# TinyMPC/TinyMPC

Hardware: AMD Instinct MI355X
Metric: QP solves/sec (+ ADMM iters/sec), 64k-batch quadrotor hover (higher is better)
Workload: dtype f64; 1 GPU; quadrotor_hovering (nx=12, nu=4, N=10), 65536 identical instances per GPU, closed-loop MPC steps from a cold start (BASELINE configs[1]); batch_per_gpu=65536, total_batch=65536, parallelism=batch-sharded x1, mpc_steps_per_launch=8, stats_exchange=none (one rank), launcher=plain process

## Files before the change

tinympc_amd/csrc/admm_kernel.hip.h:

```cpp
#pragma once
#include <hip/hip_runtime.h>
#include <stdint.h>

namespace tinympc_amd {

enum : int {
    TAB_MB = 0,
    TAB_MF1 = 256,
    TAB_MF2 = 512,
    TAB_PT = 768,
    TAB_VEC = 1024,
    TAB_BOUNDS = 1024 + 16 * 16,
};
enum : int {
    VEC_CB = 0,
    VEC_CF = 1,
    VEC_QR = 2,
    VEC_SMASK = 3,
    VEC_NIM = 4,
    VEC_SOCFLAG = 5,
    VEC_CONE_BASE = 6,
    VEC_CONE_MU = 7,
    VEC_LINFLAG = 9,
    VEC_TLINFLAG = 10,
// ... 133 lines not shown
        ring1<0, NA>(a0, srcA, mA);
        ring1<NA, NB>(a0, srcB, mB);
        return a0;
    } else {
        double a0 = init, a1 = 0.0;
        ring<MODE, 0, NA>(a0, a1, srcA, mA);
        ring<MODE, NA, NB>(a0, a1, srcB, mB);
        return a0 + a1;
    }
}
template <int MODE, int COL0, int NCOL>
__device__ __forceinline__ double ring_sum(double init, double src, const double* m) {
    if constexpr (MODE == 2) {
        double a0 = init;
        ring1<COL0, NCOL>(a0, src, m);
        return a0;
    } else {
        double a0 = init, a1 = 0.0;
        ring<MODE, COL0, NCOL>(a0, a1, src, m);
        return a0 + a1;
    }
}
template <int MODE, int COL0, int NCOL>
__device__ __forceinline__ double ring_short(double init, double src, const double* m) {
    if constexpr (MODE == 1) return ring_sum<1, COL0, NCOL>(init, src, m);
    else { double a0 = init; ring1<COL0, NCOL>(a0, src, m); return a0; }
}


#define RINGH_LO(k, p) DPP_FMA("a0", "src", "m" #k, "%[c0]+" #k, "0x3")
#define RINGH_HI(k, p) DPP_FMA("a0", "src", "m" #k, "8+%[c0]+" #k, "0xc")
#define RINGH_CASE(K)                                                                                                                    \
    if constexpr (NCOL == K)                                                                                                             \
        asm("s_nop 1\n\t" DPP_REP(K, RINGH_LO) "s_nop 0\n\t" DPP_REP(K, RINGH_HI) : [a0] "+&v"(a0) : [src] "v"(src), [c0] "i"(COL0) DPP_REP(K, DPP_ROW_M));
template <int COL0, int NCOL>
__device__ __forceinline__ void ring1_half(double& a0, double src, const double* m) {
    static_assert(NCOL >= 1 && COL0 + NCOL <= 8, "one half row");
    RINGH_CASE(1) RINGH_CASE(2) RINGH_CASE(3) RINGH_CASE(4) RINGH_CASE(5) RINGH_CASE(6) RINGH_CASE(7) RINGH_CASE(8)
}


#if defined(TINYMPC_FUSED_NX) && defined(TINYMPC_FUSED_NU)
#define TINYMPC_FUSED 1
constexpr bool fused_shape(int na, int nb) { return na == TINYMPC_FUSED_NX && nb == TINYMPC_FUSED_NU; }
#define FUSED_ROW_OPERANDS [c0] "i"(TINYMPC_FUSED_NX) DPP_REP(TINYMPC_FUSED_NX, DPP_ROW_A) DPP_REP(TINYMPC_FUSED_NU, DPP_ROW_B)
#else
constexpr bool fused_shape(int, int) { return false; }
#endif
#define BWD_COL_A(k, p) DPP_FMA("acc", "sa", "a" #k, #k, "0xf")
#define BWD_COL_B(k, p) DPP_FMA("acc", "sb", "b" #k, "%[c0]+" #k, "0xf")
#define FWD_COL_A(k, p) DPP_FMA("t", "xi", "a" #k, #k, "0xf")
#define FWD_COL_B(k, p) DPP_FMA("xn", "t", "b" #k, "%[c0]+" #k, "0xf")
#define FWD_COL_B_INPLACE(k, p) DPP_FMA("t", "t", "b" #k, "%[c0]+" #k, "%[bm]")
template <int NA, int NB>
__device__ __forceinline__ void fused_backward_step(double& qlo, double& acc, double vn, double g, double qx, double rho, double smask, double cb,
                                                    double sa, double sb, const double* ma, const double* mb_) {
#ifdef TINYMPC_FUSED
    if constexpr (fused_shape(NA, NB)) {
        double tmp;
        asm("v_add_f64 %[tmp], %[vn], -%[g]\n\t"
            "v_fma_f64 %[qlo], -%[rho], %[tmp], %[qx]\n\t"
            "v_fma_f64 %[acc], %[qlo], %[smask], %[cb]\n\t"
            DPP_REP(TINYMPC_FUSED_NX, BWD_COL_A) DPP_REP(TINYMPC_FUSED_NU, BWD_COL_B)
            : [qlo] "=&v"(qlo), [acc] "=&v"(acc), [tmp] "=&v"(tmp)
            : [vn] "v"(vn), [g] "v"(g), [qx] "v"(qx), [rho] "v"(rho), [smask] "v"(smask), [cb] "v"(cb), [sa] "v"(sa), [sb] "v"(sb), FUSED_ROW_OPERANDS);
    }
#endif
}
template <int NA, int NB>
__device__ __forceinline__ void fused_backward_step_soc(double& qlo, double& acc, double vn, double g, double qx, double w, double rho,
                                                        double smask, double cb, double sa, double sb, const double* ma, const double* mb_) {
#ifdef TINYMPC_FUSED
    if constexpr (fused_shape(NA, NB)) {
        double tmp;
        asm("v_add_f64 %[tmp], %[vn], -%[g]\n\t"
            "v_fma_f64 %[qlo], -%[rho], %[tmp], %[qx]\n\t"
            "v_fma_f64 %[qlo], -%[rho], %[w], %[qlo]\n\t"
            "v_fma_f64 %[acc], %[qlo], %[smask], %[cb]\n\t"
            DPP_REP(TINYMPC_FUSED_NX, BWD_COL_A) DPP_REP(TINYMPC_FUSED_NU, BWD_COL_B)
            : [qlo] "=&v"(qlo), [acc] "=&v"(acc), [tmp] "=&v"(tmp)
            : [vn] "v"(vn), [g] "v"(g), [qx] "v"(qx), [rho] "v"(rho), [smask] "v"(smask), [cb] "v"(cb), [sa] "v"(sa), [sb] "v"(sb),
              [w] "v"(w), FUSED_ROW_OPERANDS);
    }
#endif
}
template <int NA, int NB, bool INPLACE = false>
__device__ __forceinline__ void fused_forward_step(double& tt, double& vn, double& t, double& xn, double xi, double g, double lo, double hi,
                                                   const double* ma, const double* mb_) {
#ifdef TINYMPC_FUSED
    if constexpr (fused_shape(NA, NB) && !(INPLACE && TINYMPC_FUSED_NX % 4 == 0)) {
        double vm;
        asm("v_add_f64 %[tt], %[xi], %[g]\n\t"
            "v_max_f64 %[vm], %[lo], %[tt]\n\t"
            DPP_REP(TINYMPC_FUSED_NX, FWD_COL_A)
            "v_min_f64 %[vn], %[hi], %[vm]\n\t"
            "v_mov_b64 %[xn], %[t]\n\t"
            DPP_REP(TINYMPC_FUSED_NU, FWD_COL_B)
            : [tt] "=&v"(tt), [vm] "=&v"(vm), [vn] "=&v"(vn), [xn] "=&v"(xn), [t] "+&v"(t)
            : [xi] "v"(xi), [g] "v"(g), [lo] "v"(lo), [hi] "v"(hi), FUSED_ROW_OPERANDS);
    }
    if constexpr (fused_shape(NA, NB) && INPLACE && TINYMPC_FUSED_NX % 4 == 0) {
        asm("v_add_f64 %[tt], %[xi], %[g]\n\t"
            DPP_REP(TINYMPC_FUSED_NX, FWD_COL_A)
            "v_max_f64 %[vn], %[lo], %[tt]\n\t"
            "v_min_f64 %[vn], %[hi], %[vn]\n\t"
            DPP_REP(TINYMPC_FUSED_NU, FWD_COL_B_INPLACE)
            : [tt] "=&v"(tt), [vn] "=&v"(vn), [t] "+&v"(t)
            : [xi] "v"(xi), [g] "v"(g), [lo] "v"(lo), [hi] "v"(hi), [bm] "i"((1 << (TINYMPC_FUSED_NX / 4)) - 1), FUSED_ROW_OPERANDS);
        xn = t;
    }
#endif
}
#if defined(TINYMPC_FUSED) && TINYMPC_FUSED_NX + TINYMPC_FUSED_NU <= 8
#define TINYMPC_FUSED_HALF 1
#endif
#define HBWD_COL_A_LO(k, p) DPP_FMA("acc", "sa", "a" #k, #k, "0x3")
#define HBWD_COL_A_HI(k, p) DPP_FMA("acc", "sa", "a" #k, "8+" #k, "0xc")
#define HBWD_COL_B_LO(k, p) DPP_FMA("acc", "sb", "b" #k, "%[c0]+" #k, "0x3")
// ... 5 lines not shown
template <int NA, int NB>
__device__ __forceinline__ void fused_backward_step_half(double& qlo, double& acc, double& dnp, double& tmpn, double tmp, double vnn, double gn, double qx,
                                                         double rho, double smask, double cb, double nim, double cf, double sa, double sb,
                                                         const double* ma, const double* mb_) {
#ifdef TINYMPC_FUSED_HALF
    if constexpr (fused_shape(NA, NB)) {
        asm("v_fma_f64 %[qlo], -%[rho], %[tmp], %[qx]\n\t"
            "v_fma_f64 %[acc], %[qlo], %[smask], %[cb]\n\t"
            "v_fma_f64 %[dnp], %[sa], %[nim], %[cf]\n\t"
            DPP_REP(TINYMPC_FUSED_NX, HBWD_COL_A_LO) DPP_REP(TINYMPC_FUSED_NU, HBWD_COL_B_LO)
            "v_add_f64 %[tmpn], %[vnn], -%[gn]\n\t"
            DPP_REP(TINYMPC_FUSED_NX, HBWD_COL_A_HI) DPP_REP(TINYMPC_FUSED_NU, HBWD_COL_B_HI)
            : [qlo] "=&v"(qlo), [acc] "=&v"(acc), [dnp] "=&v"(dnp), [tmpn] "=&v"(tmpn)
            : [tmp] "v"(tmp), [vnn] "v"(vnn), [gn] "v"(gn), [qx] "v"(qx), [rho] "v"(rho), [smask] "v"(smask), [cb] "v"(cb),
              [nim] "v"(nim), [cf] "v"(cf), [sa] "v"(sa), [sb] "v"(sb), FUSED_ROW_OPERANDS);
    }
#endif
}
template <int NA, int NB>
__device__ __forceinline__ void fused_forward_step_half(double& tt, double& vn, double& t, double& xn, double& gnew, double xi, double g,
                                                        double lo, double hi, const double* ma, const double* mb_) {
#ifdef TINYMPC_FUSED_HALF
    if constexpr (fused_shape(NA, NB)) {
        double vm;
        asm("v_add_f64 %[tt], %[xi], %[g]\n\t"
            "v_max_f64 %[vm], %[lo], %[tt]\n\t"
            DPP_REP(TINYMPC_FUSED_NX, HFWD_COL_A_LO)
            "v_min_f64 %[vn], %[hi], %[vm]\n\t"
            DPP_REP(TINYMPC_FUSED_NX, HFWD_COL_A_HI)
            "v_mov_b64 %[xn], %[t]\n\t"
            "v_add_f64 %[gnew], %[tt], -%[vn]\n\t"
            DPP_REP(TINYMPC_FUSED_NU, HFWD_COL_B_LO)
            "s_nop 0\n\t"
            DPP_REP(TINYMPC_FUSED_NU, HFWD_COL_B_HI)
            : [tt] "=&v"(tt), [vm] "=&v"(vm), [vn] "=&v"(vn), [xn] "=&v"(xn), [t] "+&v"(t), [gnew] "=&v"(gnew)
            : [xi] "v"(xi), [g] "v"(g), [lo] "v"(lo), [hi] "v"(hi), FUSED_ROW_OPERANDS);
    }
#endif
}

__device__ __forceinline__ double vmax64(double a, double b) {
    double r;
    asm("v_max_f64 %0, %1, %2" : "=v"(r) : "v"(a), "v"(b));
    return r;
}
__device__ __forceinline__ double vmin64(double a, double b) {
    double r;
    asm("v_min_f64 %0, %1, %2" : "=v"(r) : "v"(a), "v"(b));
    return r;
}
__device__ __forceinline__ double pinned_sub64(double a, double b) {
    double r = a - b;
    asm volatile("" : "+v"(r));
    return r;
}
__device__ __forceinline__ double vclamp64(double lo, double hi, double t) {
    double r;
    asm("v_max_f64 %0, %1, %2\n\tv_min_f64 %0, %3, %0" : "=&v"(r) : "v"(lo), "v"(t), "v"(hi));
    return r;
}

__device__ __forceinline__ double vmax_abs64(double a, double b) {
    double r;
    asm("v_max_f64 %0, %1, |%2|" : "=v"(r) : "v"(a), "v"(b));
    return r;
}
template <bool OPAQUE>
__device__ __forceinline__ double resid_max(double a, double b) {
    if constexpr (OPAQUE) return vmax_abs64(a, b);
    else return fmax(a, fabs(b));
}

#ifndef TINYMPC_PRIM_STORE
#define TINYMPC_PRIM_STORE 1
#endif
#ifndef TINYMPC_REF_LOAD
#define TINYMPC_REF_LOAD 1
#endif
#ifndef TINYMPC_FULL_LINE_STORES
#define TINYMPC_FULL_LINE_STORES 2
#endif
__device__ __forceinline__ double load_ref(const double* p) {
#if TINYMPC_REF_LOAD == 1
    return __builtin_nontemporal_load(p);
#else
    return *p;
#endif
}
__device__ __forceinline__ void store_primal(double* p, double v) {
#if TINYMPC_PRIM_STORE == 1
    __builtin_nontemporal_store(v, p);
#elif TINYMPC_PRIM_STORE == 2
    asm volatile("global_store_dwordx2 %0, %1, off sc1" : : "v"(p), "v"(v) : "memory");
#elif TINYMPC_PRIM_STORE == 3
    asm volatile("global_store_dwordx2 %0, %1, off sc0 sc1" : : "v"(p), "v"(v) : "memory");
#elif TINYMPC_PRIM_STORE == 4
    asm volatile("global_store_dwordx2 %0, %1, off sc0 sc1 nt" : : "v"(p), "v"(v) : "memory");
#else
    *p = v;
#endif
}

__device__ __forceinline__ double grp_max16(double v) {
#pragma unroll
    for (int off = 8; off >= 1; off >>= 1) v = fmax(v, __shfl_xor(v, off, 16));
    return v;
// ... 169 lines not shown
        socmask = P.tab[TAB_VEC + VEC_SOCFLAG * 16 + j];
        soc_lane = socmask != 0.0;
        cone_base = (int)P.tab[TAB_VEC + VEC_CONE_BASE * 16 + j];
        cone_c = (cone_base >= 0) ? (j - cone_base) : 0;
        proj_lane = soc_lane && cone_base >= 0;
    }
    constexpr int SOC_PASSES = SOC ? (soc_item_passes(NX, NU, N) > 0 ? soc_item_passes(NX, NU, N) : 1) : 1;
    int item_at[SOC_PASSES];
    float item_mu[SOC_PASSES], item_rmu[SOC_PASSES];
    bool mu_pow2 = true;
    int soc_passes = 0;
    if constexpr (SOC) {
        if (lane < 3) {
            sC[4 * N * SLOT_D + lane] = lane == 2 ? 1.0 : 0.0;
            sC[4 * N * SLOT_D + PL_GC + lane] = 0.0;
            sC[4 * N * SLOT_D + PL_VC + lane] = lane == 2 ? 1.0 : 0.0;
        }
        const unsigned heads = (unsigned)(__builtin_amdgcn_ballot_w64(proj_lane && cone_c == 0) & 0xFFFFull);
#pragma unroll
        for (int p = 0; p < SOC_PASSES; ++p) {
            int t = p * 16 + j;
            item_at[p] = 4 * N * SLOT_D; item_mu[p] = 1.0f;
            if (heads && p * 16 < soc_items_of(heads, NX, N)) soc_passes = p + 1;
            for (unsigned m = heads; m; m &= m - 1) {
                const int hb = __builtin_ctz(m);
                const int cnt = hb < NX ? N : N - 1;
                if (t >= 0 && t < cnt) {
                    item_at[p] = (grp * N + t + (hb < NX ? 0 : 1)) * SLOT_D + hb;
                    item_mu[p] = (float)P.tab[TAB_VEC + VEC_CONE_MU * 16 + hb];
                    t = -1;
                } else if (t >= 0) t -= cnt;
            }
            item_rmu[p] = 1.0f / item_mu[p];
            const unsigned mb_ = __float_as_uint(item_mu[p]);
            const bool p2 = (mb_ & 0x807FFFFFu) == 0u && (mb_ >> 23) >= 127u - 60u && (mb_ >> 23) <= 127u + 60u;
            if (__builtin_amdgcn_ballot_w64(!p2) != 0ull) mu_pow2 = false;
        }
    }
    bool lin_lane = false, tlin_lane = false;
    if constexpr (LS) lin_lane = P.tab[TAB_VEC + VEC_LINFLAG * 16 + j] != 0.0;
    if constexpr (LT) tlin_lane = P.tab[TAB_VEC + VEC_TLINFLAG * 16 + j] != 0.0;
    constexpr bool LPL = solve_kernel_lin_planes(NX, NU, N, SOC, LIN, KMAX, UB);
    constexpr bool LSP = LS && LPL, LTP = LT && LPL, LSR = LS && !LPL, LTR = LT && !LPL;
    constexpr int CSL = LPL ? ((NZ + 1) | 1) : 1;
    __shared__ double sLV[LSP ? 4 * N * CSL : 1], sLG[LSP ? 4 * N * CSL : 1];
    __shared__ double sTV[LTP ? 4 * N * CSL : 1], sTG[LTP ? 4 * N * CSL : 1];
    double ones[(LSR || LTR) ? 16 : 1];
#pragma unroll
    for (int k = 0; k < ((LSR || LTR) ? 16 : 1); ++k) ones[k] = 1.0;
    bool lin_x_on = false, lin_u_on = false, tlin_x_on = false, tlin_u_on = false;
    if constexpr (LS) { lin_x_on = P.tab[TAB_VEC + VEC_LINFLAG * 16] != 0.0; lin_u_on = P.tab[TAB_VEC + VEC_LINFLAG * 16 + NX] != 0.0; }
    if constexpr (LT) { tlin_x_on = P.tab[TAB_VEC + VEC_TLINFLAG * 16] != 0.0; tlin_u_on = P.tab[TAB_VEC + VEC_TLINFLAG * 16 + NX] != 0.0; }
    double rho = P.rho;
    __builtin_amdgcn_fence(__ATOMIC_RELEASE, "wavefront");
    __builtin_amdgcn_wave_barrier();

    const double lo_u = P.tab[TAB_BOUNDS + (N > 1 ? 16 : 0) + j], hi_u = P.tab[TAB_BOUNDS + N * 16 + (N > 1 ? 16 : 0) + j];
    const double lo_u0 = P.tab[TAB_BOUNDS + j], hi_u0 = P.tab[TAB_BOUNDS + N * 16 + j];
    const int ninst = PF ? P.batch : (P.index ? *P.count : (P.perm ? P.perm_count : P.batch));
    const int ntiles = (ninst + IPW - 1) / IPW;
    const bool resumed = !PF && P.index != nullptr;
    const bool has_traj = !PF && P.traj != nullptr;
    extern __shared__ __attribute__((aligned(16))) double sPF[];
    typedef const __attribute__((address_space(1))) void* pf_gptr;
    typedef __attribute__((address_space(3))) void* pf_lptr;
    constexpr int PF_S0 = 128, PF_S1 = PF_S0 + PF_ARR, PF_S2 = PF_S1 + PF_ARR, PF_S3 = PF_S2 + PF_ARR;
    auto pf_issue = [&](const int t) {
        const int tl = P.reverse ? ntiles - 1 - t : t;
        __builtin_amdgcn_global_load_lds((pf_gptr)(P.x0 + ((size_t)tl * (IPW * NX) + (size_t)lane * 2)), (pf_lptr)sPF, 16, 0, 0);
        const size_t t0 = (size_t)tl * (IPW * RECD) + (size_t)lane * 2;
        auto arr = [&](const double* p, const int at) {
#pragma unroll
            for (int q = 0; q < PF_PIECES; ++q) __builtin_amdgcn_global_load_lds((pf_gptr)(p + t0 + q * 128), (pf_lptr)(sPF + at + q * 128), 16, 0, 0);
        };
        if (!P.cold) { arr(P.slack, PF_S0); arr(P.dual, PF_S1); arr(P.slack_prev, PF_S2); }
        if (P.pf_mask & 8) arr(P.ref, P.cold ? PF_S0 : PF_S3);
    };
    unsigned pf_ticket = 0u;
    const int pf_shard = PF ? (int)(blockIdx.x % (unsigned)(P.pf_shards > 0 ? P.pf_shards : 1)) : 0;
    typedef __attribute__((address_space(1))) unsigned* pf_ctr_t;
    unsigned long long pf_ctr_bits = PF ? (unsigned long long)(P.pf_counter + 16 * pf_shard) : 0ull;
    if constexpr (PF) asm volatile("" : "+v"(pf_ctr_bits));
    const pf_ctr_t pf_ctr = (pf_ctr_t)pf_ctr_bits;
    auto pf_draw = [&]() { return lane == 0 ? __hip_atomic_fetch_add(pf_ctr, 1u, __ATOMIC_RELAXED, __HIP_MEMORY_SCOPE_AGENT) : 0u; };
    const unsigned pf_base = PF ? P.pf_base[pf_shard] : 0u;
    int pf_next = 0, pf_i = 0;
    bool pf_first = true;
    double* const sQX = sPF + PF_S3;
    if constexpr (PF) {
        if ((int)blockIdx.x < ntiles) {
            pf_issue((int)blockIdx.x);
            if (P.pf_static <= 1) pf_ticket = pf_draw();
        }
        if (P.ref_shared) {
            double rl = 0.0, qxs[N];
#pragma unroll
            for (int s = 0; s < N; ++s) {
                const bool valid = is_state || (is_input && s >= 1);
                const double r = valid ? P.ref[j - (is_input ? NZ : 0) + s * NZ] : 0.0;
                qxs[s] = -(r * qr);
                if (s == N - 1) rl = r;
            }
            double pt[NX];
#pragma unroll
            for (int k = 0; k < NX; ++k) pt[k] = sPt[k * 16 + j];
            double xp = 0.0;
// ... 27 lines not shown
            const int lrow = grp * RECD + (j < NZ ? j - (is_input ? NZ : 0) : 0);
            const bool warm_t = !P.cold;
            pf_x0 = sPF[grp * NX + (is_state ? j : 0)];
#pragma unroll
            for (int s = 0; s < N; ++s) { pfVN[s] = 0.0; pfG[s] = 0.0; pfVP[s] = 0.0; }
            if (warm_t) {
#pragma unroll
                for (int s = 0; s < N; ++s) { pfVN[s] = sPF[PF_S0 + lrow + s * NZ]; pfG[s] = sPF[PF_S1 + lrow + s * NZ]; }
            }
            auto own_ref = [&](const int at) {
#pragma unroll
                for (int s = 0; s < N; ++s) {
                    const bool valid = is_state || (is_input && s >= 1);
                    const double r = valid ? sPF[at + lrow + s * NZ] : 0.0;
                    pfQXs[s] = -(r * qr);
                    if (s == N - 1) pf_rl = r;
                }
            };
            if (m & 8) { if (warm_t) own_ref(PF_S3); else own_ref(PF_S0); }
            else {
#pragma unroll
                for (int s = 0; s < N; ++s) pfQXs[s] = sQX[s * 16 + j];
            }
            if (warm_t) {
#pragma unroll
                for (int s = 0; s < N; ++s) pfVP[s] = sPF[PF_S2 + lrow + s * NZ];
            }
            asm volatile("s_waitcnt lgkmcnt(0)" ::: "memory");
            if (pf_next < ntiles) {
                if (pf_i + 2 >= P.pf_static) {
                    asm volatile("" ::: "memory");
                    pf_ticket = pf_draw();
                }
                pf_issue(pf_next);
            }
            ++pf_i;
        }
        (void)pfVN; (void)pfG; (void)pfVP; (void)pf_rl; (void)pf_x0; (void)pfQXs; (void)pf_first; (void)pf_ticket; (void)sQX; (void)pf_ctr; (void)pf_base; (void)pf_draw; (void)pf_i;
        if (slot < ninst) {
            const int b = PF ? slot : (resumed ? P.index[slot] : (P.perm ? P.perm[slot] : slot));
            const double* het = nullptr;
            if constexpr (HET) {
                het = P.het_tabs + (size_t)b * TAB_BOUNDS;
#pragma unroll
                for (int k = 0; k < NZ; ++k) mb[k] = het[TAB_MB + k * 16 + j];
#pragma unroll
                for (int k = 0; k < NX; ++k) mf1[k] = het[TAB_MF1 + k * 16 + j];
#pragma unroll
                for (int k = 0; k < NU; ++k) mf2[k] = het[TAB_MF2 + (NX + k) * 16 + j];
                cb = het[TAB_VEC + VEC_CB * 16 + j];
                cf = het[TAB_VEC + VEC_CF * 16 + j];
                qr = het[TAB_VEC + VEC_QR * 16 + j];
                rho = het[TAB_VEC + 8 * 16 + j];
            }
            if constexpr (ADAPT) {
                rho = P.arho[b];
                const double* aK = P.aK + (size_t)b * (NU * NX);
                if (is_state) {
#pragma unroll
                    for (int k = 0; k < NU; ++k) mb[NX + k] = -aK[k + NU * j];
#pragma unroll
                    for (int k = 0; k < NX; ++k) sP[grp * NX * NX + k + NX * j] = P.aP[(size_t)b * (NX * NX) + k + NX * j];
                } else if (is_input) {
#pragma unroll
                    for (int k = 0; k < NX; ++k) mf1[k] = -aK[(j - NX) + NU * k];
                }
                __builtin_amdgcn_fence(__ATOMIC_RELEASE, "wavefront");
                __builtin_amdgcn_wave_barrier();
            }
            const double* atab_i = nullptr;
            if constexpr (HET && ADAPT) atab_i = P.atab + (size_t)b * ATAB_DOUBLES;
            (void)atab_i;
            const size_t lbase = (size_t)b * (N * NZ) + j - (is_input ? NZ : 0);
            double X[N], G[N], VN[N], VP[N], QX[N], Dn[N - 1];
            const int cw = grp * N * SLOT_D + (j < NZ ? j : NZ);
            const double x0v_in = is_state ? (PF ? pf_x0 : P.x0[(size_t)b * NX + j]) : 0.0;
            const int cl = grp * N * CSL + (j < NZ ? j : NZ);
            double VL[LSR ? N : 1], GL[LSR ? N : 1], VT[LTR ? N : 1], GT[LTR ? N : 1];
            double Qd[DBG ? N : 1], Pd[DBG ? N : 1], Dd[DBG ? N : 1];
            double ref_last = 0.0, qx_last_plain = 0.0;
#pragma unroll
            for (int s = 0; s < N; ++s) {
                const bool valid = is_state || (is_input && s >= 1);
                const size_t off = lbase + s * NZ;
                const bool warm = valid && !P.cold;
                if constexpr (PF) {
                    VN[s] = warm ? pfVN[s] : 0.0;
                    G[s] = warm ? pfG[s] : 0.0;
                    VP[s] = warm ? pfVP[s] : 0.0;
                    QX[s] = pfQXs[s];
                    X[s] = 0.0;
                    if (s == N - 1) ref_last = pf_rl;
                    continue;
                }
                const double r = valid ? (P.ref_shared ? P.ref[off - (size_t)b * (N * NZ)] : load_ref(P.ref + off)) : 0.0;
                VN[s] = warm ? P.slack[off] : 0.0;
                G[s] = warm ? P.dual[off] : 0.0;
                VP[s] = warm ? P.slack_prev[off] : 0.0;
                QX[s] = -(r * qr);
                X[s] = 0.0;
                if (s == N - 1) ref_last = r;
                if constexpr (SOC) {
                    double vc0 = (warm && soc_lane) ? (resumed ? P.cslack : P.prim)[off] : 0.0;
                    const double gc0 = (warm && soc_lane) ? P.cdual[off] : 0.0;
                    if (s == 0 && is_state && soc_lane && !resumed) vc0 = x0v_in;
                    sC[cw + s * SLOT_D] = vc0 - gc0;
// ... 59 lines not shown
            const int traj_k0 = has_traj ? (P.traj_step0 + (P.traj_offsets ? P.traj_offsets[b] : 0)) : 0;

            int iter = 0, solved = 0, checked = 0;
            unsigned acc_iter = 0, acc_solved = 0;
            bool vp_touched = false;
            double rp = 0.0, rd = 0.0;
            const int nsteps = PF ? 1 : (P.steps > 1 ? P.steps : 1);
            const int iter_first = resumed ? P.iter_base : 0;
            for (int step = 0; step < nsteps; ++step) {
                X[0] = x0v;
                if (has_traj) {
                    if (is_state) {
#pragma unroll
                        for (int s = 0; s < N; ++s) {
                            int kk = traj_k0 + step + s;
                            kk = kk < P.traj_points ? kk : P.traj_points - 1;
                            const double r = P.traj[(size_t)kk * NX + j];
                            QX[s] = -(r * qr);
                            if (s == N - 1) ref_last = r;
                        }
                    }
                    terminal_term();
                }
                if (P.reset_duals) {
#pragma unroll
                    for (int s = 0; s < N; ++s) G[s] = 0.0;
                }
                if constexpr (SOC) {
                    if (step > 0) {
#pragma unroll
                        for (int s = 0; s < N; ++s) {
                            const double vc0 = soc_lane ? X[s] : 0.0;
                            sC[cw + s * SLOT_D] = vc0 - sC[cw + s * SLOT_D + PL_GC];
                            sC[cw + s * SLOT_D + PL_VC] = vc0;
                        }
                    }
                }
                if constexpr (LS) {
                    if (step > 0) {
#pragma unroll
                        for (int s = 0; s < N; ++s) { if constexpr (LSP) sLV[cl + s * CSL] = lin_lane ? X[s] : 0.0; else VL[s] = lin_lane ? X[s] : 0.0; }
                    } else if (is_state && lin_lane && !resumed) { if constexpr (LSP) sLV[cl] = x0v; else VL[0] = x0v; }
                }
                if constexpr (LT) {
                    if (step > 0) {
#pragma unroll
                        for (int s = 0; s < N; ++s) { if constexpr (LTP) sTV[cl + s * CSL] = tlin_lane ? X[s] : 0.0; else VT[s] = tlin_lane ? X[s] : 0.0; }
                    } else if (is_state && tlin_lane && !resumed) { if constexpr (LTP) sTV[cl] = x0v; else VT[0] = x0v; }
                }
                if constexpr (LPL) __builtin_amdgcn_fence(__ATOMIC_RELEASE, "wavefront");
                const int iter0 = iter_first;
                iter = iter0; solved = 0;
                if (resumed && P.check_termination > 0) checked = 1;
                int countdown = P.check_termination;
                double wr[SOC ? SPR : 1];
                bool gcz[SOC_PASSES];
#pragma unroll
                for (int p = 0; p < SOC_PASSES; ++p) gcz[p] = false;
                if constexpr (SOC) {
#pragma unroll
                    for (int d = 1; d <= SPR && d <= N; ++d) wr[(N - d) % SPR] = sC[cw + (N - d) * SLOT_D];
                }
                for (int it = iter0; it < P.max_iter; ++it) {
                    double lvr[LSP ? SPR : 1], lgr[LSP ? SPR : 1], tvr[LTP ? SPR : 1], tgr[LTP ? SPR : 1];
                    if constexpr (LPL) {
#pragma unroll
                        for (int d = 1; d <= SPR && d <= N; ++d) {
                            if constexpr (LSP) { lvr[(N - d) % SPR] = sLV[cl + (N - d) * CSL]; lgr[(N - d) % SPR] = sLG[cl + (N - d) * CSL]; }
                            if constexpr (LTP) { tvr[(N - d) % SPR] = sTV[cl + (N - d) * CSL]; tgr[(N - d) % SPR] = sTG[cl + (N - d) * CSL]; }
                        }
                    }
                    auto lin_w = [&](const int s_) { if constexpr (LSP) return lvr[s_ % SPR] - lgr[s_ % SPR]; else return VL[LSR ? s_ : 0] - GL[LSR ? s_ : 0]; };
                    auto tlin_w = [&](const int s_) { if constexpr (LTP) return tvr[s_ % SPR] - tgr[s_ % SPR]; else return VT[LTR ? s_ : 0] - GT[LTR ? s_ : 0]; };
                    double qhi;
                    {
                        double t = fma(-rho, VN[N - 1] - G[N - 1], QX[N - 1]);
                        if constexpr (SOC) t = fma(-rho, wr[(N - 1) % SPR], t);
                        if constexpr (LS) t = fma(-rho, lin_w(N - 1), t);
                        if constexpr (LT) t = fma(-rho, tlin_w(N - 1), t);
                        qhi = t;
                        if constexpr (DBG) {
                            double ql = fma(-rho, VN[N - 1] - G[N - 1], qx_last_plain);
                            if constexpr (SOC) ql = fma(-rho, wr[(N - 1) % SPR], ql);
                            if constexpr (LS) ql = fma(-rho, lin_w(N - 1), ql);
                            if constexpr (LT) ql = fma(-rho, tlin_w(N - 1), ql);
                            Qd[N - 1] = is_state ? ql : t;
                            Pd[N - 1] = t;
                        }
                    }
                    double pcur = qhi;
                    if constexpr (HALF) {
                        double tmpv = VN[N - 2] - G[N - 2];
#pragma unroll
                        for (int i = N - 2; i >= 0; --i) {
                            double qlo, res, dnp, tmpn;
                            constexpr int dummy = 0;
                            const int in = i > 0 ? i - 1 : dummy;
                            fused_backward_step_half<NX, NU>(qlo, res, dnp, tmpn, tmpv, VN[in], G[in], QX[i], rho, smask, cb, nim, cf, pcur, qhi, mb, mb + NX);
                            if (i + 1 <= N - 2) Dn[i + 1] = dnp;
                            tmpv = tmpn;
                            pcur = res;
                            qhi = qlo;
                        }
                        Dn[0] = fma(pcur, nim, cf);
                    }
#pragma unroll
                    for (int i = N - 2; i >= 0 && !HALF; --i) {
                        if constexpr (SOC) {
                            if (i >= SPD) wr[(i - SPD) % SPR] = sC[cw + (i - SPD) * SLOT_D];
                        }
                        if constexpr (LSP) { if (i >= SPD) { lvr[(i - SPD) % SPR] = sLV[cl + (i - SPD) * CSL]; lgr[(i - SPD) % SPR] = sLG[cl + (i - SPD) * CSL]; } }
                        if constexpr (LTP) { if (i >= SPD) { tvr[(i - SPD) % SPR] = sTV[cl + (i - SPD) * CSL]; tgr[(i - SPD) % SPR] = sTG[cl + (i - SPD) * CSL]; } }
                        if constexpr (SOC || LPL) __builtin_amdgcn_sched_barrier(0);
                        if constexpr (FUSED) {
                            double qlo, res;
                            if constexpr (SOC) fused_backward_step_soc<NX, NU>(qlo, res, VN[i], G[i], QX[i], wr[i % SPR], rho, smask, cb, pcur, qhi, mb, mb + NX);
                            else fused_backward_step<NX, NU>(qlo, res, VN[i], G[i], QX[i], rho, smask, cb, pcur, qhi, mb, mb + NX);
                            pcur = res;
                            Dn[i] = fma(res, nim, cf);
                            if constexpr (DBG) { Qd[i] = qlo; Pd[i] = res; Dd[i + 1] = res; }
                            qhi = qlo;
                            continue;
                        }
                        double qlo = fma(-rho, VN[i] - G[i], QX[i]);
                        if constexpr (SOC) qlo = fma(-rho, wr[i % SPR], qlo);
                        if constexpr (LS) qlo = fma(-rho, lin_w(i), qlo);
                        if constexpr (LT) qlo = fma(-rho, tlin_w(i), qlo);
                        const double res = ring_sum2<MODE, NX, NU>(fma(qlo, smask, cb), pcur, mb, qhi, mb + NX);
                        pcur = res;
                        Dn[i] = fma(res, nim, cf);
                        if constexpr (DBG) { Qd[i] = qlo; Pd[i] = res; Dd[i + 1] = res; }
                        qhi = qlo;
                    }
                    constexpr bool LAZY_RES = N <= 12;
                    constexpr bool TIGHT = FUSED && !HALF && LAZY_RES && !SOC && NX % 4 == 0;
                    double pmax = 0.0, dmax = 0.0;
                    auto slot_update = [&](const int s, const double lo, const double hi, const double gcv, const double glv, const double gtv) {
                        const double xi = X[s];
                        const double t = xi + G[s];
                        const double vn = TIGHT ? vclamp64(lo, hi, t) : vmin64(hi, vmax64(lo, t));
                        if constexpr (!LAZY_RES) {
                            pmax = resid_max<true>(pmax, xi - vn);
                            dmax = resid_max<true>(dmax, VP[s] - vn);
                        }
                        G[s] = t - vn;
                        VN[s] = vn;
                        if constexpr (SOC) {
                            sC[cw + s * SLOT_D] = fma(xi, socmask, gcv);
                        }
                        if constexpr (LSP) sLV[cl + s * CSL] = (lin_lane && (is_state || s >= 1)) ? (xi + glv) : 0.0;
                        if constexpr (LTP) sTV[cl + s * CSL] = (tlin_lane && (is_state || s >= 1)) ? (xi + gtv) : 0.0;
                        if constexpr (LSR || LTR) {
                            auto halfspaces = [&](double z, const double* tabk, const int nk) {
                                for (int k = 0; k < nk; ++k) {
                                    const double a = tabk[k * 16 + j];
                                    const double bk = tabk[KMAX * 16 + k * 16 + j];
                                    const double nn = tabk[2 * KMAX * 16 + k * 16 + j];
                                    const double prod = a * z;
                                    double cs = 0.0, ci = 0.0;
                                    ring1<0, NX>(cs, prod, ones);
                                    ring1<NX, NU>(ci, prod, ones);
                                    const double cv = is_state ? cs : ci;
                                    if (cv > bk) z = z - ((cv - bk) / nn) * a;
                                }
                                return z;
                            };
                            if constexpr (LSR) {
                                const bool on = lin_lane && (is_state || s >= 1);
                                double vl = on ? (xi + GL[s]) : 0.0;
                                vl = halfspaces(vl, sLin, P.n_lin);
                                GL[s] = on ? ((GL[s] + xi) - vl) : 0.0;
                                VL[s] = on ? vl : 0.0;
                            }
                            if constexpr (LTR) {
                                const bool on = tlin_lane && (is_state || s >= 1);
                                double vt = on ? (xi + GT[s]) : 0.0;
                                vt = halfspaces(vt, sTLin + s * 3 * KMAX * 16, P.n_tlin);
                                GT[s] = on ? ((GT[s] + xi) - vt) : 0.0;
                                VT[s] = on ? vt : 0.0;
                            }
                        }
                    };
                    double lo_c = UB ? lo_u0 : sLo[j], hi_c = UB ? hi_u0 : sHi[j];
                    double gr[SOC ? SPR : 1];
                    if constexpr (SOC) {
#pragma unroll
                        for (int d = 0; d < SPD && d < N; ++d) gr[d % SPR] = sC[cw + d * SLOT_D + PL_GC];
                    } else gr[0] = 0.0;
                    double glr[LSP ? SPR : 1], gtr[LTP ? SPR : 1];
                    glr[0] = 0.0; gtr[0] = 0.0;
                    if constexpr (LPL) {
#pragma unroll
                        for (int d = 0; d < SPD && d < N; ++d) {
                            if constexpr (LSP) glr[d % SPR] = sLG[cl + d * CSL];
                            if constexpr (LTP) gtr[d % SPR] = sTG[cl + d * CSL];
                        }
                    }
                    double tt_d = 0.0, vn_d = 0.0;
#pragma unroll
                    for (int i = 0; i < N - 1; ++i) {
                        const double lo_n = UB ? lo_u : sLo[(i + 1) * 16 + j], hi_n = UB ? hi_u : sHi[(i + 1) * 16 + j];
                        if constexpr (SOC) { if (i + SPD < N) gr[(i + SPD) % SPR] = sC[cw + (i + SPD) * SLOT_D + PL_GC]; }
                        if constexpr (LSP) { if (i + SPD < N) glr[(i + SPD) % SPR] = sLG[cl + (i + SPD) * CSL]; }
                        if constexpr (LTP) { if (i + SPD < N) gtr[(i + SPD) % SPR] = sTG[cl + (i + SPD) * CSL]; }
                        __builtin_amdgcn_sched_barrier(0);
                        if constexpr (FUSED) {
                            double tt, vn, xn, t = Dn[i];
                            const double xi = X[i];
                            if constexpr (HALF) {
                                double gnew;
                                fused_forward_step_half<NX, NU>(tt, vn, t, xn, gnew, xi, G[i], lo_c, hi_c, mf1, mf2);
                                X[i + 1] = xn;
                                if constexpr (!LAZY_RES) {
                                    pmax = resid_max<true>(pmax, xi - vn);
                                    dmax = resid_max<true>(dmax, VP[i] - vn);
                                }
                                G[i] = gnew;
                                VN[i] = vn;
                                lo_c = lo_n; hi_c = hi_n;
                                continue;
                            }
                            fused_forward_step<NX, NU, TIGHT>(tt, vn, t, xn, xi, G[i], lo_c, hi_c, mf1, mf2);
                            X[i + 1] = xn;
                            if constexpr (!LAZY_RES) {
                                pmax = resid_max<true>(pmax, xi - vn);
                                dmax = resid_max<true>(dmax, VP[i] - vn);
                            }
                            if constexpr (TIGHT) {
                                __builtin_amdgcn_sched_barrier(0);
                                if (i > 0) G[i - 1] = pinned_sub64(tt_d, vn_d);
                                tt_d = tt; vn_d = vn;
                            } else G[i] = tt - vn;
                            VN[i] = vn;
                            if constexpr (SOC) sC[cw + i * SLOT_D] = fma(xi, socmask, gr[i % SPR]);
                            lo_c = lo_n; hi_c = hi_n;
                            continue;
                        }
                        const double t = ring_sum<MODE, 0, NX>(Dn[i], X[i], mf1);
                        X[i + 1] = ring_short<MODE, NX, NU>(t, t, mf2);
                        slot_update(i, lo_c, hi_c, gr[SOC ? i % SPR : 0], glr[LSP ? i % SPR : 0], gtr[LTP ? i % SPR : 0]);
                        lo_c = lo_n; hi_c = hi_n;
                    }
                    if constexpr (TIGHT && N >= 2) G[N - 2] = tt_d - vn_d;
                    (void)tt_d; (void)vn_d;
                    slot_update(N - 1, lo_c, hi_c, gr[SOC ? (N - 1) % SPR : 0], glr[LSP ? (N - 1) % SPR : 0], gtr[LTP ? (N - 1) % SPR : 0]);
                    if constexpr (LPL) {
                        __builtin_amdgcn_fence(__ATOMIC_RELEASE, "wavefront");
                        __builtin_amdgcn_wave_barrier();
                        if constexpr (LSP) {
                            if (lin_x_on) project_halfspace_columns<NX, KMAX, 16, 16>(j, grp, N, CSL, 0, 0, sLV, sLG, sLin, 0, P.n_lin);
                            if (lin_u_on) project_halfspace_columns<NU, KMAX, 16, 16>(j, grp, N, CSL, NX, 1, sLV, sLG, sLin, 0, P.n_lin);
                        }
                        if constexpr (LTP) {
                            if (tlin_x_on) project_halfspace_columns<NX, KMAX, 16, 16>(j, grp, N, CSL, 0, 0, sTV, sTG, sTLin, 3 * KMAX * 16, P.n_tlin);
                            if (tlin_u_on) project_halfspace_columns<NU, KMAX, 16, 16>(j, grp, N, CSL, NX, 1, sTV, sTG, sTLin, 3 * KMAX * 16, P.n_tlin);
                        }
                        __builtin_amdgcn_fence(__ATOMIC_RELEASE, "wavefront");
                        __builtin_amdgcn_wave_barrier();
                    }
                    bool conv = false;
                    auto termination = [&]() {
                        if (countdown > 0 && --countdown == 0) {
                            countdown = P.check_termination;
                            checked = 1;
                            constexpr int PS0 = N >= 2 ? 1 : 0, PS1 = N - 1;
                            auto lost = [&](const int s) {
                                return (int)(fabs(X[s] - VN[s]) >= P.tol_pri) | (int)(fabs(VP[s] - VN[s]) * rho >= P.tol_dua);
                            };
                            const bool maybe = ((int)!(rho > 0.0) | (int)!(lost(PS0) | lost(PS1))) != 0;
                            unsigned long long fold = __ballot(maybe);
                            fold &= fold >> 1; fold &= fold >> 2; fold &= fold >> 4;
                            if constexpr (!HALF) fold &= fold >> 8;
                            const bool any_row = (fold & (HALF ? 0x0101010101010101ull : 0x0001000100010001ull)) != 0ull;
                            const bool last_test = (P.max_iter - 1 - it) < P.check_termination;
                            if (last_test || any_row) {
                                if constexpr (LAZY_RES) {
#pragma unroll
                                    for (int s = 0; s < N; ++s) {
                                        pmax = resid_max<false>(pmax, X[s] - VN[s]);
                                        dmax = resid_max<false>(dmax, VP[s] - VN[s]);
                                    }
                                }
                                rp = pmax;
                                rd = dmax * rho;
                                const bool ok = (rp < P.tol_pri) && (rd < P.tol_dua);
                                const unsigned long long bal = __ballot(ok);
                                conv = ((bal >> (grp * RL)) & RMASK) == RMASK;
                            }
                        }
                    };
                    if constexpr (SOC) {
                        __builtin_amdgcn_fence(__ATOMIC_RELEASE, "wavefront");
                        __builtin_amdgcn_wave_barrier();
                        double n0 = sC[item_at[0]], n1 = sC[item_at[0] + 1], n2 = sC[item_at[0] + 2];
#pragma unroll
                        for (int d = 1; d <= SPR && d <= N; ++d) wr[(N - d) % SPR] = sC[cw + (N - d) * SLOT_D];
                        termination();
                        bool any_exact = false;
#pragma unroll
                        for (int p = 0; p < SOC_PASSES; ++p) {
                            if (p > 0 && p >= soc_passes) break;
                            const int at = item_at[p];
                            if (p > 0) { n0 = sC[at]; n1 = sC[at + 1]; n2 = sC[at + 2]; }
                            const double s0 = n0, s1 = n1, s2 = n2;
                            if (soc_all_inside(s0, s1, s2, item_mu[p])) {
                                sC[at + PL_VC] = s0; sC[at + PL_VC + 1] = s1; sC[at + PL_VC + 2] = s2;
                                if (!gcz[p]) {
                                    sC[at + PL_GC] = 0.0; sC[at + PL_GC + 1] = 0.0; sC[at + PL_GC + 2] = 0.0;
                                    gcz[p] = true;
                                }
                            } else {
                                double r0, r1, r2;
                                soc_project3(s0, s1, s2, item_mu[p], item_rmu[p], mu_pow2, r0, r1, r2);
                                const double g0 = s0 - r0, g1 = s1 - r1, g2 = s2 - r2;
                                sC[at + PL_VC] = r0; sC[at + PL_VC + 1] = r1; sC[at + PL_VC + 2] = r2;
                                sC[at + PL_GC] = g0; sC[at + PL_GC + 1] = g1; sC[at + PL_GC + 2] = g2;
                                sC[at] = r0 - g0; sC[at + 1] = r1 - g1; sC[at + 2] = r2 - g2;
                                gcz[p] = false;
                                any_exact = true;
                            }
                        }
                        if (it == iter0 && !proj_lane) {
#pragma unroll
                            for (int s = 0; s < N; ++s) sC[cw + s * SLOT_D + PL_GC] = 0.0;
                        }
                        __builtin_amdgcn_fence(__ATOMIC_RELEASE, "wavefront");
                        __builtin_amdgcn_wave_barrier();
                        if (any_exact) {
// ... 24 lines not shown
                                const double xs = is_state ? X[i] : X[i + 1];
                                const double px = qr * xs;
                                dual_res = fmax(dual_res, on ? fabs((px + px) + aty) : 0.0);
                                pxq_max = fmax(pxq_max, on ? fabs(px) : 0.0);
                                aty_max = fmax(aty_max, on ? fabs(aty) : 0.0);
                            }
                            {
                                double prow[NX];
#pragma unroll
                                for (int k = 0; k < NX; ++k) prow[k] = sP[grp * NX * NX + (is_state ? j : 0) + NX * k];
                                const double pxl = ring_sum<MODE, 0, NX>(0.0, X[N - 1], prow);
                                const double ql = qr * X[N - 1];
                                const double atyl = -G[N - 1];
                                dual_res = fmax(dual_res, is_state ? fabs((pxl + ql) + atyl) : 0.0);
                                px_max = fmax(pxq_max, is_state ? fabs(pxl) : 0.0);
                                aty_max = fmax(aty_max, is_state ? fabs(atyl) : 0.0);
                                q_max = fmax(pxq_max, is_state ? fabs(ql) : 0.0);
                            }
                            pri_res = grp_max16(pri_res); ax_max = grp_max16(ax_max); z_max = grp_max16(z_max);
                            dual_res = grp_max16(dual_res); px_max = grp_max16(px_max); aty_max = grp_max16(aty_max); q_max = grp_max16(q_max);
                            const double pri_norm = fmax(ax_max, z_max);
                            const double dual_norm = fmax(fmax(px_max, aty_max), q_max);
                            const double eps = 1e-10;
                            const double normalized_pri = pri_res / (pri_norm + eps);
                            const double normalized_dual = dual_res / (dual_norm + eps);
                            const double ratio = normalized_pri / (normalized_dual + eps);
                            double new_rho = rho * sqrt(ratio);
                            if (P.aclip) new_rho = fmin(fmax(new_rho, P.arho_min), P.arho_max);
                            const double delta = new_rho - rho;
                            if (is_state) {
#pragma unroll
                                for (int k = 0; k < NU; ++k) mb[NX + k] = -taylor_step(-mb[NX + k], delta, (HA ? atab_i[ATAB_DK + k * 16 + j] : sTab[(16 + j) * AKC + k]));
#pragma unroll
                                for (int k = 0; k < NX; ++k) {
                                    const int e = grp * NX * NX + k + NX * j;
                                    sP[e] = taylor_step(sP[e], delta, (HA ? atab_i[ATAB_DP + k * 16 + j] : sTab[(32 + j) * AKC + k]));
                                }
                            } else if (is_input) {
#pragma unroll
                                for (int k = 0; k < NX; ++k) mf1[k] = -taylor_step(-mf1[k], delta, (HA ? atab_i[ATAB_DK + k * 16 + j] : sTab[(16 + j) * AKC + k]));
                            }
                            if (P.aC1 || P.aC2) {
                                if (j == 0) sDl[grp * ADAPT_LOG + ndl] = delta;
                                if (++ndl == ADAPT_LOG) { flush_c(ndl); ndl = 0; }
                            }
                            rho = new_rho;
                            __builtin_amdgcn_fence(__ATOMIC_RELEASE, "wavefront");
                            __builtin_amdgcn_wave_barrier();
                            QX[N - 1] = qx_last_plain;
                            terminal_term();
                        }
                    }
                    if constexpr (!SOC) termination();
                    if (conv) { solved = 1; break; }
#pragma unroll
                    for (int s = 0; s < N; ++s) VP[s] = VN[s];
                    vp_touched = true;
                }
                acc_iter += (unsigned)(iter - iter0);
                acc_solved += (unsigned)solved;
                if (P.iter_log && j == 0) P.iter_log[(size_t)step * P.batch + b] = solved ? iter : -iter;
                if (P.u0_log && is_input) P.u0_log[((size_t)step * P.batch + b) * NU + (j - NX)] = X[1];
                if (nsteps > 1) {
                    x0v = is_state ? X[1] : 0.0;
                }
            }

            constexpr bool FLS = TINYMPC_FULL_LINE_STORES != 0 && (PF || TINYMPC_FULL_LINE_STORES == 2) && !SOC && LIN == 0 && !DBG;
            if (FLS && (P.store_mask & 32) == 0) {
                if constexpr (FLS) {
                    const size_t seg = (size_t)b * (N * NZ) + j;
                    const bool in_row = j < NZ;
#pragma unroll
                    for (int s = 0; s < N; ++s) {
                        const size_t off = seg + s * NZ;
                        const double xs = is_input ? (s + 1 < N ? X[s + 1 < N ? s + 1 : s] : 0.0) : X[s];
                        const double vs = is_input ? (s + 1 < N ? VN[s + 1 < N ? s + 1 : s] : 0.0) : VN[s];
                        const double gs = is_input ? (s + 1 < N ? G[s + 1 < N ? s + 1 : s] : 0.0) : G[s];
                        const double ps = is_input ? (s + 1 < N ? VP[s + 1 < N ? s + 1 : s] : 0.0) : VP[s];
                        if (in_row) {
                            if (P.store_mask & 1) {
                                if (acc_iter > 0) { if constexpr (PF) P.prim[off] = xs; else store_primal(P.prim + off, xs); }
                                else if (s == 0 && is_state) P.prim[off] = xs;
                            }
                            if (P.store_mask & 2) P.slack[off] = vs;
                            if (P.store_mask & 4) P.dual[off] = gs;
                            if ((P.store_mask & 8) && vp_touched) P.slack_prev[off] = ps;
                        }
                    }
                }
            } else
#pragma unroll
            for (int s = 0; s < N; ++s) {
                const bool valid = is_state || (is_input && s >= 1);
                const size_t off = lbase + s * NZ;
                if (valid) {
                    if (((P.store_mask & 1) || ((P.store_mask & 32) && s <= 1)) && (acc_iter > 0 || (s == 0 && is_state))) {
                        if constexpr (SOC || LIN != 0) P.prim[off] = X[s];
                        else store_primal(P.prim + off, X[s]);
                    }
                    if (P.store_mask & 2) P.slack[off] = VN[s];
                    if (P.store_mask & 4) P.dual[off] = G[s];
                    if ((P.store_mask & 8) && vp_touched) P.slack_prev[off] = VP[s];
                    if constexpr (SOC) {
                        if (soc_lane && (P.store_mask & 16)) {
                            P.cslack[off] = sC[cw + s * SLOT_D + ((proj_lane || iter <= iter_first) ? PL_VC : 0)];
                            P.cdual[off] = sC[cw + s * SLOT_D + PL_GC];
                        }
                    }
                    if constexpr (LSP) { if (lin_lane && (P.store_mask & 16)) { P.lslack[off] = sLV[cl + s * CSL]; P.ldual[off] = sLG[cl + s * CSL]; } }
                    if constexpr (LTP) { if (tlin_lane && (P.store_mask & 16)) { P.tlslack[off] = sTV[cl + s * CSL]; P.tldual[off] = sTG[cl + s * CSL]; } }
// ... 56 lines not shown
```

Baseline: 2.903 billion QP solves/s.

## Precompute dual threshold, probe termination early, and skip VP copies in tight kernel

For the tight fused non-adaptive path, the change precomputes a wave-uniform dual tolerance threshold (tol_dua/rho) in scalar registers. The termination probe can then use ballots directly instead of multiplying by rho per lane. It moves the cheap convergence probe into the forward pass at slot 1 and defers the VP copy for slots 2..N-1 to the rare full-check or loop-exit case, cutting per-iteration register moves. It also pins rho as a scalar operand in the backward asm, and skews the Dn fma by one step so it overlaps with the DPP chain. The risks are subtle changes to termination semantics, since the probe now checks only one slot, and added register pressure and code complexity.

```diff
diff --git a/tinympc_amd/csrc/admm_kernel.hip.h b/tinympc_amd/csrc/admm_kernel.hip.h
--- a/tinympc_amd/csrc/admm_kernel.hip.h
+++ b/tinympc_amd/csrc/admm_kernel.hip.h
@@ -209,11 +209,21 @@
 #define FWD_COL_A(k, p) DPP_FMA("t", "xi", "a" #k, #k, "0xf")
 #define FWD_COL_B(k, p) DPP_FMA("xn", "t", "b" #k, "%[c0]+" #k, "0xf")
 #define FWD_COL_B_INPLACE(k, p) DPP_FMA("t", "t", "b" #k, "%[c0]+" #k, "%[bm]")
-template <int NA, int NB>
+template <int NA, int NB, bool RHO_S = false>
 __device__ __forceinline__ void fused_backward_step(double& qlo, double& acc, double vn, double g, double qx, double rho, double smask, double cb,
-                                                    double sa, double sb, const double* ma, const double* mb_) {
+                                                    double sa, double sb, const double* ma, const double* mb_, double* tmp_keep = nullptr) {
 #ifdef TINYMPC_FUSED
-    if constexpr (fused_shape(NA, NB)) {
+    if constexpr (fused_shape(NA, NB) && RHO_S) {
+        double tmp;
+        asm("v_add_f64 %[tmp], %[vn], -%[g]\n\t"
+            "v_fma_f64 %[qlo], -%[rho], %[tmp], %[qx]\n\t"
+            "v_fma_f64 %[acc], %[qlo], %[smask], %[cb]\n\t"
+            DPP_REP(TINYMPC_FUSED_NX, BWD_COL_A) DPP_REP(TINYMPC_FUSED_NU, BWD_COL_B)
+            : [qlo] "=&v"(qlo), [acc] "=&v"(acc), [tmp] "=&v"(tmp)
+            : [vn] "v"(vn), [g] "v"(g), [qx] "v"(qx), [rho] "s"(rho), [smask] "v"(smask), [cb] "v"(cb), [sa] "v"(sa), [sb] "v"(sb), FUSED_ROW_OPERANDS);
+        if (tmp_keep) *tmp_keep = tmp;
+    }
+    if constexpr (fused_shape(NA, NB) && !RHO_S) {
         double tmp;
         asm("v_add_f64 %[tmp], %[vn], -%[g]\n\t"
             "v_fma_f64 %[qlo], -%[rho], %[tmp], %[qx]\n\t"
@@ -221,6 +231,7 @@
             DPP_REP(TINYMPC_FUSED_NX, BWD_COL_A) DPP_REP(TINYMPC_FUSED_NU, BWD_COL_B)
             : [qlo] "=&v"(qlo), [acc] "=&v"(acc), [tmp] "=&v"(tmp)
             : [vn] "v"(vn), [g] "v"(g), [qx] "v"(qx), [rho] "v"(rho), [smask] "v"(smask), [cb] "v"(cb), [sa] "v"(sa), [sb] "v"(sb), FUSED_ROW_OPERANDS);
+        if (tmp_keep) *tmp_keep = tmp;
     }
 #endif
 }
@@ -332,6 +343,11 @@
 __device__ __forceinline__ double pinned_sub64(double a, double b) {
     double r = a - b;
     asm volatile("" : "+v"(r));
+    return r;
+}
+__device__ __forceinline__ double pinned_fma64(double a, double b, double c, double keep) {
+    double r = fma(a, b, c);
+    asm volatile("" : "+v"(r) : "v"(keep));
     return r;
 }
 __device__ __forceinline__ double vclamp64(double lo, double hi, double t) {
@@ -607,6 +623,22 @@
     if constexpr (LS) { lin_x_on = P.tab[TAB_VEC + VEC_LINFLAG * 16] != 0.0; lin_u_on = P.tab[TAB_VEC + VEC_LINFLAG * 16 + NX] != 0.0; }
     if constexpr (LT) { tlin_x_on = P.tab[TAB_VEC + VEC_TLINFLAG * 16] != 0.0; tlin_u_on = P.tab[TAB_VEC + VEC_TLINFLAG * 16 + NX] != 0.0; }
     double rho = P.rho;
+    constexpr bool TIGHTK = FUSED && !HALF && N <= 12 && !SOC && NX % 4 == 0;
+    constexpr bool THR = TIGHTK && !ADAPT;
+    double thr = 0.0;
+    unsigned long long rho_bad = 0ull;
+    auto form_thr = [&]() {
+        const double q = P.tol_dua / rho;
+        thr = (q >= 0x1p-1000 && q < __builtin_huge_val()) ? q * (1.0 + 0x1p-50) : __builtin_nan("");
+        rho_bad = __builtin_amdgcn_ballot_w64(!(rho > 0.0));
+        if constexpr (!HET) {
+            const unsigned long long tb = (unsigned long long)__double_as_longlong(thr);
+            const unsigned tl = __builtin_amdgcn_readfirstlane((unsigned)tb), th = __builtin_amdgcn_readfirstlane((unsigned)(tb >> 32));
+            thr = __longlong_as_double((long long)(((unsigned long long)th << 32) | tl));
+        }
+    };
+    if constexpr (THR && !HET) form_thr();
+    (void)thr; (void)rho_bad; (void)form_thr;
     __builtin_amdgcn_fence(__ATOMIC_RELEASE, "wavefront");
     __builtin_amdgcn_wave_barrier();
 
@@ -740,6 +772,7 @@
                 cf = het[TAB_VEC + VEC_CF * 16 + j];
                 qr = het[TAB_VEC + VEC_QR * 16 + j];
                 rho = het[TAB_VEC + 8 * 16 + j];
+                if constexpr (THR) form_thr();
             }
             if constexpr (ADAPT) {
                 rho = P.arho[b];
@@ -905,6 +938,8 @@
                 const int iter0 = iter_first;
                 iter = iter0; solved = 0;
                 if (resumed && P.check_termination > 0) checked = 1;
+                if constexpr (TIGHTK) { if (P.check_termination > 0 && P.max_iter - iter0 >= P.check_termination) checked = 1; }
+                bool left = false;
                 int countdown = P.check_termination;
                 double wr[SOC ? SPR : 1];
                 bool gcz[SOC_PASSES];
@@ -957,6 +992,8 @@
                         }
                         Dn[0] = fma(pcur, nim, cf);
                     }
+                    double res_d = 0.0;
+                    (void)res_d;
 #pragma unroll
                     for (int i = N - 2; i >= 0 && !HALF; --i) {
                         if constexpr (SOC) {
@@ -966,11 +1003,18 @@
                         if constexpr (LTP) { if (i >= SPD) { tvr[(i - SPD) % SPR] = sTV[cl + (i - SPD) * CSL]; tgr[(i - SPD) % SPR] = sTG[cl + (i - SPD) * CSL]; } }
                         if constexpr (SOC || LPL) __builtin_amdgcn_sched_barrier(0);
                         if constexpr (FUSED) {
-                            double qlo, res;
+                            double qlo, res, tmp_k = 0.0;
+                            (void)tmp_k;
                             if constexpr (SOC) fused_backward_step_soc<NX, NU>(qlo, res, VN[i], G[i], QX[i], wr[i % SPR], rho, smask, cb, pcur, qhi, mb, mb + NX);
-                            else fused_backward_step<NX, NU>(qlo, res, VN[i], G[i], QX[i], rho, smask, cb, pcur, qhi, mb, mb + NX);
+                            else fused_backward_step<NX, NU, TIGHTK && !HET && !ADAPT>(qlo, res, VN[i], G[i], QX[i], rho, smask, cb, pcur, qhi, mb, mb + NX,
+                                                                                        (THR && N >= 3) ? &tmp_k : nullptr);
                             pcur = res;
-                            Dn[i] = fma(res, nim, cf);
+                            if constexpr (THR && N >= 3) {
+                                __builtin_amdgcn_sched_barrier(0);
+                                if (i < N - 2) Dn[i + 1] = pinned_fma64(res_d, nim, cf, tmp_k);
+                                res_d = res;
+                                if (i == 0) Dn[0] = fma(res, nim, cf);
+                            } else Dn[i] = fma(res, nim, cf);
                             if constexpr (DBG) { Qd[i] = qlo; Pd[i] = res; Dd[i + 1] = res; }
                             qhi = qlo;
                             continue;
@@ -987,6 +1031,7 @@
                     }
                     constexpr bool LAZY_RES = N <= 12;
                     constexpr bool TIGHT = FUSED && !HALF && LAZY_RES && !SOC && NX % 4 == 0;
+                    static_assert(TIGHT == TIGHTK, "the one-slot probe and the loop's scalar bookkeeping belong to the TIGHT form");
                     double pmax = 0.0, dmax = 0.0;
                     auto slot_update = [&](const int s, const double lo, const double hi, const double gcv, const double glv, const double gtv) {
                         const double xi = X[s];
@@ -1050,6 +1095,22 @@
                         }
                     }
                     double tt_d = 0.0, vn_d = 0.0;
+                    constexpr bool EARLY = THR && N >= 3;
+                    bool full_due = false;
+                    auto early_probe = [&]() {
+                        if (countdown == 1) {
+                            const unsigned long long lost_p = __builtin_amdgcn_ballot_w64(fabs(X[1] - VN[1]) >= P.tol_pri);
+                            const unsigned long long lost_d = __builtin_amdgcn_ballot_w64(fabs(VP[1] - VN[1]) >= thr);
+                            unsigned long long fold = (~(lost_p | lost_d) | rho_bad) & __builtin_amdgcn_ballot_w64(true);
+                            fold &= fold >> 1; fold &= fold >> 2; fold &= fold >> 4; fold &= fold >> 8;
+                            full_due = (fold & 0x0001000100010001ull) != 0ull || (P.max_iter - 1 - it) < P.check_termination;
+                            if (__builtin_expect(full_due && it > iter0, false)) {
+#pragma unroll
+                                for (int s = 2; s < N; ++s) VP[s] = VN[s];
+                            }
+                        }
+                    };
+                    (void)early_probe; (void)full_due;
 #pragma unroll
                     for (int i = 0; i < N - 1; ++i) {
                         const double lo_n = UB ? lo_u : sLo[(i + 1) * 16 + j], hi_n = UB ? hi_u : sHi[(i + 1) * 16 + j];
@@ -1085,6 +1146,7 @@
                                 tt_d = tt; vn_d = vn;
                             } else G[i] = tt - vn;
                             VN[i] = vn;
+                            if constexpr (EARLY) { if (i == 1) early_probe(); }
                             if constexpr (SOC) sC[cw + i * SLOT_D] = fma(xi, socmask, gr[i % SPR]);
                             lo_c = lo_n; hi_c = hi_n;
                             continue;
@@ -1115,18 +1177,24 @@
                     auto termination = [&]() {
                         if (countdown > 0 && --countdown == 0) {
                             countdown = P.check_termination;
-                            checked = 1;
+                            if constexpr (!TIGHTK) checked = 1;
                             constexpr int PS0 = N >= 2 ? 1 : 0, PS1 = N - 1;
                             auto lost = [&](const int s) {
                                 return (int)(fabs(X[s] - VN[s]) >= P.tol_pri) | (int)(fabs(VP[s] - VN[s]) * rho >= P.tol_dua);
                             };
-                            const bool maybe = ((int)!(rho > 0.0) | (int)!(lost(PS0) | lost(PS1))) != 0;
-                            unsigned long long fold = __ballot(maybe);
+                            unsigned long long fold = 0ull;
+                            if constexpr (EARLY) {
+                            } else if constexpr (THR) {
+                                const unsigned long long lost_p = __builtin_amdgcn_ballot_w64(fabs(X[PS0] - VN[PS0]) >= P.tol_pri);
+                                const unsigned long long lost_d = __builtin_amdgcn_ballot_w64(fabs(VP[PS0] - VN[PS0]) >= thr);
+                                fold = (~(lost_p | lost_d) | rho_bad) & __builtin_amdgcn_ballot_w64(true);
+                            } else fold = __ballot(((int)!(rho > 0.0) | (int)!(lost(PS0) | lost(PS1))) != 0);
                             fold &= fold >> 1; fold &= fold >> 2; fold &= fold >> 4;
                             if constexpr (!HALF) fold &= fold >> 8;
                             const bool any_row = (fold & (HALF ? 0x0101010101010101ull : 0x0001000100010001ull)) != 0ull;
                             const bool last_test = (P.max_iter - 1 - it) < P.check_termination;
-                            if (last_test || any_row) {
+                            const bool full_test = EARLY ? full_due : (last_test || any_row);
+                            if (TIGHTK ? __builtin_expect(full_test, false) : full_test) {
                                 if constexpr (LAZY_RES) {
 #pragma unroll
                                     for (int s = 0; s < N; ++s) {
@@ -1257,11 +1325,19 @@
                         }
                     }
                     if constexpr (!SOC) termination();
-                    if (conv) { solved = 1; break; }
-#pragma unroll
-                    for (int s = 0; s < N; ++s) VP[s] = VN[s];
+                    if (conv) { if constexpr (TIGHTK) left = true; else solved = 1; break; }
+#pragma unroll
+                    for (int s = 0; s < N; ++s) { if (!EARLY || s < 2) VP[s] = VN[s]; }
                     vp_touched = true;
                 }
+                if constexpr (TIGHTK) solved = left ? 1 : 0;
+                if constexpr (THR && N >= 3) {
+                    if (!left && P.max_iter > iter0) {
+#pragma unroll
+                        for (int s = 2; s < N; ++s) VP[s] = VN[s];
+                    }
+                }
+                (void)left;
                 acc_iter += (unsigned)(iter - iter0);
                 acc_solved += (unsigned)solved;
                 if (P.iter_log && j == 0) P.iter_log[(size_t)step * P.batch + b] = solved ? iter : -iter;
```

Measured after the change: 2.834 billion QP solves/s. 2.4% lower.
